# tataganesh/Query-Efficient-Approx-to-improve-OCR

Hardware: AMD Instinct MI355X
Metric: patch-images/sec UNet->CRNN->CTC fwd+bwd, 32x128 grey (higher is better)
Workload: dtype f32 (GEMMs as scaled 2 x fp16 split products — three fp16 MFMAs per fp32 multiply-add — fp32 accumulate); 1 GPU; BASELINE configs[2]: full minibatch step of train_nn_area.py:212-287 — Phase A (UNet eval fwd, TopKCER k = 5 % of the minibatch, inner_limit = 4 jitter replicas fused in the batch dim, CRNN train-BN fwd+bwd, Adam(CRNN)) + Phase B (UNet train-BN -> CRNN BN-eval -> CTC mean + MSE -> backward -> Adam(UNet)) + greedy decode -> CER -> update_cer (:290-304) on synthetic POS-style 32x128 patches; batch_per_gpu=2048, global_batch=2048, full_step=True, crnn_wgrad=True, parallelism=dp1, hipgraph=False

## Files before the change

query-efficient-approx-to-improve-ocr_amd/csrc/conv_igemm.hip:

```cpp
#include "conv_args.h"
#include <string>
#include <type_traits>
#include <stdlib.h>
#include <string.h>

using qea_conv::ConvArgs;
using qea_conv::conv_epilogue;

namespace {

template <int A_LD, int B_LD, int BK, int RPP>
struct IgemmGather {
  int lrow, kc, ntaps;
  int a_pix[A_LD];
  int a_ih0[A_LD], a_iw0[A_LD];
  const float* b_ptr[B_LD > 0 ? B_LD : 1];
  f32x4 a_reg[A_LD], b_reg[B_LD > 0 ? B_LD : 1];

  __device__ __forceinline__ void init(const ConvArgs& p, int tid, int m0, int n0) {
    constexpr int KCH = BK / 4;
    lrow = tid / KCH;
    kc = tid % KCH;
    ntaps = p.KH * p.KW;
    const int ohw = p.OH * p.OW;
#pragma unroll
    for (int i = 0; i < A_LD; ++i) {
      const int m = m0 + lrow + RPP * i;
      if (m < p.M) {
        const int b = m / ohw;
        const int rem = m - b * ohw;
        const int oh = rem / p.OW;
        const int ow = rem - oh * p.OW;
        a_pix[i] = b * p.H * p.W;
        a_ih0[i] = oh * p.stride_h - p.pad_h;
        a_iw0[i] = ow * p.stride_w - p.pad_w;
      } else {
        a_pix[i] = -1;
        a_ih0[i] = 0;
        a_iw0[i] = 0;
      }
    }
#pragma unroll
    for (int j = 0; j < B_LD; ++j) {
      const int n = n0 + lrow + RPP * j;
      b_ptr[j] = (n < p.N) ? (p.w + (size_t)n * p.K + kc * 4) : nullptr;
    }
  }

  __device__ __forceinline__ void fetch(const ConvArgs& p, int kt) {
    const int cs = kt / ntaps;
    const int tap = kt - cs * ntaps;
    const int c0 = cs * BK;
    const int kh = tap / p.KW;
    const int kw = tap - kh * p.KW;
#pragma unroll
    for (int i = 0; i < A_LD; ++i) {
      const int ih = a_ih0[i] + kh, iw = a_iw0[i] + kw;
      const bool ok = (a_pix[i] >= 0) && ((unsigned)ih < (unsigned)p.H) && ((unsigned)iw < (unsigned)p.W);
      f32x4 v = {0.f, 0.f, 0.f, 0.f};
      if (ok) v = *reinterpret_cast<const f32x4*>(p.x + (size_t)(a_pix[i] + ih * p.W + iw) * p.ldx + c0 + kc * 4);
      a_reg[i] = v;
    }
    const int koff = tap * p.Cin + c0;
#pragma unroll
    for (int j = 0; j < B_LD; ++j) {
      f32x4 v = {0.f, 0.f, 0.f, 0.f};
      if (b_ptr[j]) v = *reinterpret_cast<const f32x4*>(b_ptr[j] + koff);
      b_reg[j] = v;
    }
  }
};

template <int MI, int NJ>
__device__ __forceinline__ void zero_acc(f32x16 (&acc)[MI][NJ]) {
#pragma unroll
  for (int i = 0; i < MI; ++i)
#pragma unroll
    for (int j = 0; j < NJ; ++j)
#pragma unroll
      for (int r = 0; r < 16; ++r) acc[i][j][r] = 0.f;
}

constexpr int ROWB = 16;
// ... 646 lines not shown
#pragma unroll
        for (int i = 0; i < MI; ++i)
#pragma unroll
          for (int j = 0; j < NJ; ++j)
            acc[i][j] = __builtin_amdgcn_mfma_f32_32x32x2f32(af[i][s], bq[cur][kb][j][s], acc[i][j], 0, 0, 0);
    }
  }

  float esc[NJ], ebi[NJ];
#pragma unroll
  for (int j = 0; j < NJ; ++j) {
    esc[j] = scale ? scale[j * 32 + fr] : 1.f;
    ebi[j] = bias ? bias[j * 32 + fr] : 0.f;
  }
  double st0[NJ], st1[NJ];
  if (STATS) {
#pragma unroll
    for (int j = 0; j < NJ; ++j) st0[j] = st1[j] = 0.0;
  }
  float am = 0.f;
#pragma unroll
  for (int i = 0; i < MI; ++i) {
    float* yrow = y + ((size_t)(b * H + y0 + wave * MI + i) * W + x0) * ldy;
#pragma unroll
    for (int r = 0; r < 16; ++r) {
      const int px = (r & 3) + 8 * (r >> 2) + 4 * fh;
#pragma unroll
      for (int j = 0; j < NJ; ++j) {
        float v = acc[i][j][r];
        if (scale && bias) v = __fmaf_rn(v, esc[j], ebi[j]);
        else if (scale) v *= esc[j];
        else if (bias) v += ebi[j];
        if (relu) v = fmaxf(v, 0.f);
        yrow[(size_t)px * ldy + j * 32 + fr] = v;
        am = qea_amax_acc(am, v);
        if (STATS) {
          st0[j] += (double)v;
          st1[j] += (double)v * (double)v;
        }
      }
    }
  }
  qea_amax_commit_block(am, yamax);
  if (STATS) {
#pragma unroll
    for (int j = 0; j < NJ; ++j) {
      const double a = st0[j] + __shfl_xor(st0[j], 32, 64);
      const double c = st1[j] + __shfl_xor(st1[j], 32, 64);
      if (fh == 0) {
        double* dst = stats + ((size_t)(blockIdx.x * 4 + wave) * COUT + j * 32 + fr) * 2;
        dst[0] = a;
        dst[1] = c;
      }
    }
  }
}

template <int CIN, int COUT, int TH, bool STATS>
int launch_halo_(const ConvArgs& a, hipStream_t s) {
  constexpr size_t lds = (size_t)(TH + 2) * 34 * (CIN + 4) * sizeof(float);
  constexpr auto kern = conv3x3_halo_kernel<CIN, COUT, TH, STATS>;
  const int rc = reserve_lds<kern>("qea_conv_igemm(halo)", lds);
  if (rc != QEA_OK) return rc;
  const long long grid = (long long)a.B * (a.H / TH) * (a.W / 32);
  if (grid <= 0 || grid > 0x7fffffffLL) {
    qea_set_error("qea_conv_igemm(halo): grid %lld out of range", grid);
    return QEA_ERR_INVALID;
  }
  hipLaunchKernelGGL(kern, dim3((unsigned)grid), dim3(256), lds, s, a.x, a.w, a.y, a.B, a.H, a.W, a.ldx, a.ldy, a.scale, a.bias, a.relu, a.stats, a.yamax);
  return QEA_OK;
}

template <int CIN, int COUT, int TH>
int launch_halo(const ConvArgs& a, hipStream_t s) {
  return a.stats ? launch_halo_<CIN, COUT, TH, true>(a, s) : launch_halo_<CIN, COUT, TH, false>(a, s);
}

#ifndef QEA_HALO_NARROW_WGS
#define QEA_HALO_NARROW_WGS 3
#endif
constexpr int halo_bf3_wgs(int cin, int cout, int npl, bool bst = false) {
  return (npl == 2 && cout <= 64 && (cin == 32 || cout == 32) && !(bst && cout == 64) && QEA_HALO_NARROW_WGS == 3) ? 3 : 2;
}

template <int CIN, int COUT, int TH, bool STATS, int IMW = 0, int NPL = 3, int PKW = 0, bool BST = false>
__global__ __launch_bounds__(256) __attribute__((amdgpu_waves_per_eu(halo_bf3_wgs(CIN, COUT, NPL, BST), halo_bf3_wgs(CIN, COUT, NPL, BST)))) void conv3x3_halo_bf3_kernel(const float* __restrict__ x, const __bf16* __restrict__ wf, float* __restrict__ y,
                                                               int B, int H, int W, int ldx, int ldy, const float* __restrict__ scale,
                                                               const float* __restrict__ bias, int relu, double* __restrict__ stats, int chunks,
                                                               int Ntot, const float* __restrict__ mask, int ldmask, int total,
                                                               const float* __restrict__ xmax, float* __restrict__ yamax,
                                                               float* __restrict__ pooled, int ldp, float* __restrict__ pamax,
                                                               const float* __restrict__ yref, int ldyref, const double* __restrict__ bst64,
                                                               const float* __restrict__ bsc, const float* __restrict__ bsh) {
  constexpr bool F16 = NPL == 2;
  typedef typename std::conditional<F16, f16x8, bf16x8>::type frag_t;
  constexpr bool SMALL = IMW != 0;
  constexpr int IMH = SMALL ? IMW / 4 : 1;
  constexpr int IPX = SMALL ? 32 / IMW : 1, IPY = SMALL ? TH / IMH : 1;
  constexpr int TW = 32, HW_ = SMALL ? IPX * (IMW + 2) : TW + 2, HH = SMALL ? TH + 1 : TH + 2, HP = HH * HW_;
  static_assert(!SMALL || (TH % IMH == 0 && COUT == 128), "small-image tiles: whole images per tile, one wave row");
  constexpr int WN = COUT / 32, WM = 4 / WN;
  constexpr int MI = TH / WM;
  constexpr int KS = CIN / 16;
  constexpr int SLOTS = CIN / 8;
  constexpr int PLANE = HP * CIN;
  static_assert(MI >= 1 && TH % WM == 0, "tile rows must split over the waves");
  static_assert(PKW == 0 || (MI % 2 == 0 && !STATS && (PKW == 1 || PKW == 2)), "fused pooling: row pairs inside one wave, no statistics");
  static_assert(!BST || (!STATS && PKW == 0), "BatchNorm-backward sums: their own instances");
  extern __shared__ __attribute__((aligned(16))) float smem[];
  __bf16* As = reinterpret_cast<__bf16*>(smem);
  float sx = 1.f, inv_x = 1.f, inv_w = 1.f;
  if constexpr (F16) {
    qea_f16_scale(xmax[0], sx, inv_x);
    inv_w = reinterpret_cast<const float*>(wf + (size_t)Ntot * 9 * chunks * CIN * NPL)[0];
  }

  const int tiles_x = W / TW, tiles_y = H / TH;
  const int nblk = Ntot / COUT;
  struct Item { int nb, tile_id, b, x0, y0; };
  auto decode = [&](int vb) {
    const int lid = qea_xcd_swizzle(vb, total);
    Item it;
    it.nb = lid % nblk;
    it.tile_id = lid / nblk;
    if (SMALL) {
      it.b = it.tile_id * (IPX * IPY);
      it.x0 = it.y0 = 0;
      return it;
    }
    int bid = it.tile_id;
    const int tx = bid % tiles_x;
    bid /= tiles_x;
    const int ty = bid % tiles_y;
    it.b = bid / tiles_y;
    it.x0 = tx * TW;
    it.y0 = ty * TH;
    return it;
  };

  auto swz = [](int p, int slot) { return SLOTS == 4 ? (slot ^ ((p >> 2) & 3)) : (slot ^ ((p >> 1) & 7)); };

  constexpr int C4 = CIN / 4;
  constexpr int NLD = (HP * C4 + 255) / 256;
  f32x4 hv[NLD];
  constexpr int QS = 256 / C4;
  auto gather = [&](const Item& it, int chunk, int tid) {
    const float* xb = x + (size_t)it.b * H * W * ldx + chunk * CIN + (tid % C4) * 4;
    int q = tid / C4;
    int hy = q / HW_, hx = q - hy * HW_;
#pragma unroll
    for (int i = 0; i < NLD; ++i) {
      int iy, ix;
      bool ok;
      if (SMALL) {
        const int gx = hx / (IMW + 2);
        const int img = (hy / IMH) * IPX + gx;
        ix = hx - gx * (IMW + 2) - 1;
        iy = (img * IMH + hy % IMH);
        ok = q < HP && hy < TH && (unsigned)ix < (unsigned)IMW && it.b + img < B;
      } else {
        iy = it.y0 + hy - 1;
        ix = it.x0 + hx - 1;
        ok = q < HP && (unsigned)iy < (unsigned)H && (unsigned)ix < (unsigned)W;
      }
      const f32x4 v = *reinterpret_cast<const f32x4*>(ok ? xb + ((size_t)iy * W + ix) * ldx : x);
      const f32x4 zero = {0.f, 0.f, 0.f, 0.f};
      hv[i] = ok ? v : zero;
      q += QS;
      hx += QS;
      if (hx >= HW_) {
        hx -= HW_;
        ++hy;
      }
    }
  };
  auto stage = [&](int tid) {
    const int c4 = tid % C4;
    int q = tid / C4;
#pragma unroll
    for (int i = 0; i < NLD; ++i) {
      if (q < HP) {
        const int o = q * CIN + swz(q, c4 >> 1) * 8 + (c4 & 1) * 4;
        if constexpr (F16) {
          f16x4 h, l;
          qea_split2_f16(hv[i], sx, h, l);
          *reinterpret_cast<f16x4*>(As + o) = h;
          *reinterpret_cast<f16x4*>(As + PLANE + o) = l;
        } else {
          bf16x4 h, m, l;
          qea_split3(hv[i], h, m, l);
          *reinterpret_cast<bf16x4*>(As + o) = h;
          *reinterpret_cast<bf16x4*>(As + PLANE + o) = m;
          *reinterpret_cast<bf16x4*>(As + 2 * PLANE + o) = l;
        }
      }
      q += QS;
    }
  };

  constexpr int STEPS = 9 * KS;
  frag_t bq[2][NPL];
  auto load_b = [&](int nb, int gst, int buf, int tid) {
    const frag_t* wl = reinterpret_cast<const frag_t*>(wf) + ((tid >> 6) % WN) * 64 + (tid & 63) + (size_t)nb * chunks * STEPS * NPL * WN * 64;
#pragma unroll
    for (int pl = 0; pl < NPL; ++pl) bq[buf][pl] = wl[(size_t)(gst * NPL + pl) * WN * 64];
  };

  int vb = blockIdx.x;
  Item cur = decode(vb);
  gather(cur, 0, threadIdx.x);
  load_b(cur.nb, 0, 0, threadIdx.x);
  bool first = true;
  float am = 0.f, pm = 0.f;
  while (true) {
    const int nvb = vb + gridDim.x;
    const bool has_next = nvb < total;
    const Item nxt = decode(has_next ? nvb : vb);
    f32x16 acc[MI];
#pragma unroll
    for (int i = 0; i < MI; ++i)
#pragma unroll
      for (int r = 0; r < 16; ++r) acc[i][r] = 0.f;

    for (int chunk = 0; chunk < chunks; ++chunk) {
      int tid = threadIdx.x;
      asm volatile("" : "+v"(tid));
      const int lane = tid & 63, wave = tid >> 6;
      const int wm = wave / WN;
      const int fr = lane & 31, fh = lane >> 5;
      if (!first) __syncthreads();
      first = false;
      stage(tid);
      __syncthreads();
      if (chunk + 1 < chunks) gather(cur, chunk + 1, tid);
      else if (has_next) gather(nxt, 0, tid);
      auto read_a = [&](int st, int i, frag_t* a) {
        const int tap = st / KS, cs = st % KS;
        const int kh = tap / 3, kw = tap % 3;
        int hp;
        if (SMALL) {
          const int rr = i % IMH + kh - 1;
          const int srow = (rr >= 0 && rr < IMH) ? (i / IMH) * IMH + rr : TH;
          hp = srow * HW_ + fr + 2 * (fr / IMW) + kw;
        } else {
          hp = (wm * MI + i + kh) * HW_ + fr + kw;
        }
        const __bf16* src = As + hp * CIN + swz(hp, cs * 2 + fh) * 8;
#pragma unroll
        for (int pl = 0; pl < NPL; ++pl) a[pl] = *reinterpret_cast<const frag_t*>(src + pl * PLANE);
      };
      frag_t ar[2][NPL];
      read_a(0, 0, ar[0]);
#pragma unroll
      for (int st = 0; st < STEPS; ++st) {
        const int cb = st & 1;
        if (st + 1 < STEPS || chunk + 1 < chunks) load_b(cur.nb, chunk * STEPS + st + 1, cb ^ 1, tid);
        else if (has_next) load_b(nxt.nb, 0, cb ^ 1, tid);
        __builtin_amdgcn_sched_barrier(0);
#pragma unroll
        for (int i = 0; i < MI; ++i) {
          const int f = st * MI + i;
          const bool more = f + 1 < STEPS * MI;
          if (more) read_a((f + 1) / MI, (f + 1) % MI, ar[(f + 1) & 1]);
          acc[i] = mfma_split<NPL>(acc[i], ar[f & 1], bq[cb]);
          if (more) {
            __builtin_amdgcn_sched_group_barrier(0x100, NPL, 0);
            __builtin_amdgcn_sched_group_barrier(0x008, NPL == 2 ? 3 : 6, 0);
          }
        }
      }
    }

    int tid = threadIdx.x;
    asm volatile("" : "+v"(tid));
    const int lane = tid & 63, wave = tid >> 6;
    const int wm = wave / WN, wn = wave % WN;
    const int fr = lane & 31, fh = lane >> 5;
    const int n = cur.nb * COUT + wn * 32 + fr;
    const float esc = scale ? scale[n] : 1.f, ebi = bias ? bias[n] : 0.f;
    float msc = 0.f, msh = 0.f;
    double bmu = 0.0, bis = 0.0;
    if constexpr (BST) {
      msc = bsc[n];
      msh = bsh[n];
      bmu = bst64[n];
      bis = bst64[Ntot + n];
    }
    double st0 = 0.0, st1 = 0.0;
    if constexpr (PKW != 0) {
#pragma unroll
      for (int i = 0; i < MI; i += 2) {
        float vv[2][16];
#pragma unroll
        for (int ii = 0; ii < 2; ++ii)
#pragma unroll
          for (int r = 0; r < 16; ++r) {
            const int px = (r & 3) + 8 * (r >> 2) + 4 * fh;
            size_t prow;
            bool live = true;
            if (SMALL) {
              const int img = ((i + ii) / IMH) * IPX + px / IMW;
              prow = ((size_t)(cur.b + img) * IMH + (i + ii) % IMH) * IMW + px % IMW;
              live = cur.b + img < B;
            } else {
              prow = (size_t)(cur.b * H + cur.y0 + wm * MI + i + ii) * W + cur.x0 + px;
            }
            float v = acc[i + ii][r];
            if constexpr (F16) v = (v * inv_x) * inv_w;
            if (scale && bias) v = __fmaf_rn(v, esc, ebi);
            else if (scale) v *= esc;
            else if (bias) v += ebi;
            if (relu) v = fmaxf(v, 0.f);
            vv[ii][r] = v;
            if (!live) continue;
            y[prow * ldy + n] = v;
            am = qea_amax_acc(am, v);
          }
#pragma unroll
        for (int r = 0; r < 16; r += PKW) {
          const int px = (r & 3) + 8 * (r >> 2) + 4 * fh;
          float m = -INFINITY;
#pragma unroll
          for (int ii = 0; ii < 2; ++ii)
#pragma unroll
            for (int jj = 0; jj < PKW; ++jj) {
              const float v = vv[ii][r + jj];
              m = (v > m || v != v) ? v : m;
            }
          size_t prow;
          bool live = true;
          if (SMALL) {
            const int img = (i / IMH) * IPX + px / IMW;
            prow = ((size_t)(cur.b + img) * (IMH / 2) + (i % IMH) / 2) * (IMW / PKW) + (px % IMW) / PKW;
            live = cur.b + img < B;
          } else {
            prow = ((size_t)cur.b * (H / 2) + (cur.y0 + wm * MI + i) / 2) * (W / PKW) + (cur.x0 + px) / PKW;
          }
          if (!live) continue;
          pooled[prow * ldp + n] = m;
          pm = qea_amax_acc(pm, m);
        }
      }
    } else if constexpr (BST) {
#pragma unroll
      for (int i = 0; i < MI; ++i) {
#pragma unroll
        for (int r = 0; r < 16; ++r) {
          const int px = (r & 3) + 8 * (r >> 2) + 4 * fh;
          size_t prow;
          bool live = true;
          if (SMALL) {
            const int img = (i / IMH) * IPX + px / IMW;
            prow = ((size_t)(cur.b + img) * IMH + i % IMH) * IMW + px % IMW;
            live = cur.b + img < B;
          } else {
            prow = (size_t)(cur.b * H + cur.y0 + wm * MI + i) * W + cur.x0 + px;
          }
          float v = acc[i][r];
          if constexpr (F16) v = (v * inv_x) * inv_w;
          if (scale && bias) v = __fmaf_rn(v, esc, ebi);
          else if (scale) v *= esc;
          else if (bias) v += ebi;
          if (relu) v = fmaxf(v, 0.f);
          if (!live) continue;
          if (mask) v = (mask[prow * ldmask + n] > 0.f) ? v : 0.f;
          y[prow * ldy + n] = v;
          am = qea_amax_acc(am, v);
          const float yv = yref[prow * ldyref + n];
          const float dz = __fmaf_rn(yv, msc, msh) > 0.f ? v : 0.f;
          st0 += (double)dz;
          st1 += (double)dz * (((double)yv - bmu) * bis);
        }
      }
    } else {
      if constexpr (F16) {
#pragma unroll
        for (int i = 0; i < MI; ++i)
#pragma unroll
          for (int r = 0; r < 16; ++r) acc[i][r] = (acc[i][r] * inv_x) * inv_w;
      }
      if (scale && bias) {
#pragma unroll
        for (int i = 0; i < MI; ++i)
#pragma unroll
          for (int r = 0; r < 16; ++r) acc[i][r] = __fmaf_rn(acc[i][r], esc, ebi);
      } else if (scale) {
#pragma unroll
        for (int i = 0; i < MI; ++i)
#pragma unroll
          for (int r = 0; r < 16; ++r) acc[i][r] *= esc;
      } else if (bias) {
#pragma unroll
        for (int i = 0; i < MI; ++i)
#pragma unroll
          for (int r = 0; r < 16; ++r) acc[i][r] += ebi;
      }
      if (relu) {
#pragma unroll
        for (int i = 0; i < MI; ++i)
#pragma unroll
          for (int r = 0; r < 16; ++r) acc[i][r] = fmaxf(acc[i][r], 0.f);
      }
      auto store_rows = [&](auto has_mask) {
        constexpr bool HAS_MASK = decltype(has_mask)::value;
#pragma unroll
        for (int i = 0; i < MI; ++i) {
          const int rowpix = (cur.b * H + cur.y0 + wm * MI + i) * W + cur.x0;
          float* yb = y + (size_t)rowpix * ldy;
          const float* mb = HAS_MASK ? mask + (size_t)rowpix * ldmask : nullptr;
          const int lo = 4 * fh * ldy + n, lom = 4 * fh * ldmask + n;
#pragma unroll
          for (int r = 0; r < 16; ++r) {
            const int c = (r & 3) + 8 * (r >> 2);
            float v = acc[i][r];
            size_t prow = 0;
            if (SMALL) {
              const int px = c + 4 * fh;
              const int img = (i / IMH) * IPX + px / IMW;
              prow = ((size_t)(cur.b + img) * IMH + i % IMH) * IMW + px % IMW;
              if (cur.b + img >= B) continue;
              if (HAS_MASK) v = (mask[prow * ldmask + n] > 0.f) ? v : 0.f;
              y[prow * ldy + n] = v;
            } else {
              if (HAS_MASK) v = (mb[lom + c * ldmask] > 0.f) ? v : 0.f;
              yb[lo + c * ldy] = v;
            }
            am = qea_amax_acc(am, v);
            if (STATS) {
              st0 += (double)v;
              st1 += (double)v * (double)v;
            }
          }
        }
      };
      if (mask) store_rows(std::true_type{});
      else store_rows(std::false_type{});
    }
    if (STATS || BST) {
      const double sa = st0 + __shfl_xor(st0, 32, 64);
      const double sc = st1 + __shfl_xor(st1, 32, 64);
      if (fh == 0) {
        double* dst = stats + ((size_t)(cur.tile_id * WM + wm) * Ntot + n) * 2;
        dst[0] = sa;
        dst[1] = sc;
      }
    }
    if (!has_next) break;
    cur = nxt;
    vb = nvb;
  }
  qea_amax_commit_block(am, yamax);
  if constexpr (PKW != 0) qea_amax_commit_block(pm, pamax);
}

template <int CIN, int COUT, int TH, bool STATS, int IMW = 0, int NPL = 3, int PKW = 0, bool BST = false>
int launch_halo_bf3_(const ConvArgs& a, hipStream_t s) {
  constexpr size_t lds = IMW ? (size_t)NPL * (TH + 1) * (32 / IMW) * (IMW + 2) * CIN * 2 : (size_t)NPL * (TH + 2) * 34 * CIN * 2;
  constexpr auto kern = conv3x3_halo_bf3_kernel<CIN, COUT, TH, STATS, IMW, NPL, PKW, BST>;
  const int rc = reserve_lds<kern>("qea_conv_igemm(halo bf3)", lds);
  if (rc != QEA_OK) return rc;
  const long long total = IMW ? (long long)qea_cdiv(a.B, (32 / IMW) * (TH / (IMW / 4))) * (a.N / COUT)
                              : (long long)a.B * (a.H / TH) * (a.W / 32) * (a.N / COUT);
  if (total <= 0 || total > 0x7fffffffLL) {
    qea_set_error("qea_conv_igemm(halo bf3): grid %lld out of range", total);
    return QEA_ERR_INVALID;
  }
  const int resident = qea_persistent_grid(halo_bf3_wgs(CIN, COUT, NPL, BST));
  const unsigned grid = (total > resident && COUT > 32) ? (unsigned)resident : (unsigned)total;
  hipLaunchKernelGGL(kern, dim3(grid), dim3(256), lds, s, a.x, (const __bf16*)a.wp, a.y, a.B, a.H, a.W, a.ldx, a.ldy,
                     a.scale, a.bias, a.relu, a.stats, a.Cin / CIN, a.N, a.mask, a.ldmask, (int)total, a.xmax, a.yamax, a.pool_y, a.ldpool, a.pool_amax,
                     a.bst_y, a.ldbst, a.bst64, a.bst_scale, a.bst_shift);
  return QEA_OK;
}

template <int CIN, int COUT, int TH, int IMW = 0>
int launch_halo_bf3(const ConvArgs& a, hipStream_t s) {
  if constexpr (CIN == 32) {
    if (a.xmax && a.bst_y)
      return launch_halo_bf3_<CIN, COUT, TH, false, IMW, 2, 0, true>(a, s);
    if (a.xmax)
      return a.stats ? launch_halo_bf3_<CIN, COUT, TH, true, IMW, 2>(a, s) : launch_halo_bf3_<CIN, COUT, TH, false, IMW, 2>(a, s);
  }
  return a.stats ? launch_halo_bf3_<CIN, COUT, TH, true, IMW>(a, s) : launch_halo_bf3_<CIN, COUT, TH, false, IMW>(a, s);
}

bool halo_eligible(const qea_conv_desc* d) {
  const bool ch = (d->Cin == 32 || d->Cin == 64) && (d->N == 32 || d->N == 64);
  const int th = d->Cin == 32 ? 8 : 4;
  return ch && d->KH == 3 && d->KW == 3 && d->pad_h == 1 && d->pad_w == 1 && d->stride_h == 1 && d->stride_w == 1 && d->OH == d->H &&
         d->OW == d->W && d->W % 32 == 0 && d->H % th == 0 && d->out_mode == QEA_OUT_NHWC && !d->mask && !d->accumulate;
}

int halo_bf3_small(const qea_conv_desc* d) {
  if (d->Cin % 64 || d->Cin > 512 || d->N % 128) return 0;
  if (d->W == 16 && d->H == 4) return 16;
  if (d->W == 8 && d->H == 2) return 8;
  return 0;
}

bool halo_bf3_eligible(const qea_conv_desc* d) {
  const bool cin = d->Cin == 32 || (d->Cin % 64 == 0 && d->Cin <= 512);
  const bool cout = d->N == 32 || d->N == 64 || d->N % 128 == 0;
  const int th = d->Cin == 32 ? 8 : 4;
  const bool shape = (d->W % 32 == 0 && d->H % th == 0) || halo_bf3_small(d) != 0;
  return cin && cout && d->KH == 3 && d->KW == 3 && d->pad_h == 1 && d->pad_w == 1 && d->stride_h == 1 && d->stride_w == 1 && d->OH == d->H &&
         d->OW == d->W && shape && d->out_mode == QEA_OUT_NHWC && !d->accumulate;
}

long long halo_bf3_tiles(const qea_conv_desc* d) {
  const int sm = halo_bf3_small(d);
  if (sm) return qea_cdiv(d->B, (32 / sm) * (4 / (sm / 4)));
  return (long long)d->B * (d->H / (d->Cin == 32 ? 8 : 4)) * (d->W / 32);
}

bool halo_bf3_pool_shape(const qea_conv_desc* d, int kw) {
  if (!halo_bf3_eligible(d) || d->mask || d->stats || d->H % 2 || (kw != 1 && kw != 2) || (kw == 2 && d->W % 2)) return false;
  const int sm = halo_bf3_small(d);
  if (sm == 16) return kw == 2;
  if (sm) return false;
  if (d->Cin == 32) return d->N == 32 && kw == 2;
  if (d->N == 64) return kw == 2;
  return d->N % 128 == 0;
}

int launch_halo_bf3_any(const qea_conv_desc* d, const ConvArgs& a, hipStream_t s) {
  const int sm = halo_bf3_small(d);
  if (a.pool_y) return launch_halo_bf3_<32, 32, 8, false, 0, 2, 2>(a, s);
  if (sm == 16) return launch_halo_bf3<64, 128, 4, 16>(a, s);
  if (sm == 8) return launch_halo_bf3<64, 128, 4, 8>(a, s);
  if (d->Cin == 32) {
    if (d->N == 32) return launch_halo_bf3<32, 32, 8>(a, s);
    if (d->N == 64) return launch_halo_bf3<32, 64, 8>(a, s);
    return launch_halo_bf3<32, 128, 8>(a, s);
  }
  if (d->N == 32) return launch_halo_bf3<64, 32, 4>(a, s);
  if (d->N == 64) return launch_halo_bf3<64, 64, 4>(a, s);
  return launch_halo_bf3<64, 128, 4>(a, s);
}

int halo_bf3_wm(const qea_conv_desc* d) { return 4 / ((d->N > 128 ? 128 : d->N) / 32); }

int launch_halo_any(const qea_conv_desc* d, const ConvArgs& a, hipStream_t s) {
  if (d->Cin == 32 && d->N == 32) return launch_halo<32, 32, 8>(a, s);
  if (d->Cin == 32 && d->N == 64) return launch_halo<32, 64, 8>(a, s);
  if (d->Cin == 64 && d->N == 32) return launch_halo<64, 32, 4>(a, s);
  return launch_halo<64, 64, 4>(a, s);
}

// ... 283 lines not shown
```

Measured before the change: 22250 patch-images/s.

## Add producer-consumer warp-specialized halo conv kernel with LDS-resident filters

Adds a new 512-thread persistent kernel for 3x3 convolutions with 32 input channels, 32 or 64 output channels and 8-row tiles. Half the threads gather and stage input halos into a two-slot LDS ring with a three-deep register prefetch, while the other half run the MFMA loop and epilogue. Filter fragments are preloaded once into LDS instead of being streamed from global memory. The epilogue is factored into a shared helper. The path is taken automatically when the work exceeds one persistent wave of blocks and no pooling or BN-backward fusion is requested. It trades occupancy (one 512-thread block per CU) and extra LDS for overlap of global loads with MFMA compute.

```diff
diff --git a/query-efficient-approx-to-improve-ocr_amd/csrc/conv_igemm.hip b/query-efficient-approx-to-improve-ocr_amd/csrc/conv_igemm.hip
--- a/query-efficient-approx-to-improve-ocr_amd/csrc/conv_igemm.hip
+++ b/query-efficient-approx-to-improve-ocr_amd/csrc/conv_igemm.hip
@@ -1,4 +1,5 @@
 #include "conv_args.h"
+#include "item_walk.h"
 #include <string>
 #include <type_traits>
 #include <stdlib.h>
@@ -811,6 +812,45 @@
 constexpr int halo_bf3_wgs(int cin, int cout, int npl, bool bst = false) {
   return (npl == 2 && cout <= 64 && (cin == 32 || cout == 32) && !(bst && cout == 64) && QEA_HALO_NARROW_WGS == 3) ? 3 : 2;
 }
+
+struct HaloItem { int nb, tile_id, b, x0, y0; };
+template <int TH>
+__device__ __forceinline__ HaloItem halo_decode(int vb, int total, int nblk, int tiles_x, int tiles_y) {
+  const int lid = qea_xcd_swizzle(vb, total);
+  HaloItem it;
+  it.nb = lid % nblk;
+  it.tile_id = lid / nblk;
+  int bid = it.tile_id;
+  const int tx = bid % tiles_x;
+  bid /= tiles_x;
+  const int ty = bid % tiles_y;
+  it.b = bid / tiles_y;
+  it.x0 = tx * 32;
+  it.y0 = ty * TH;
+  return it;
+}
+template <int SLOTS>
+__device__ __forceinline__ int halo_swz(int p, int slot) { return SLOTS == 4 ? (slot ^ ((p >> 2) & 3)) : (slot ^ ((p >> 1) & 7)); }
+
+struct HaloEpilogue {
+  float* y;
+  int B, H, W, ldy;
+  const float *scale, *bias;
+  int relu;
+  double* stats;
+  int Ntot;
+  const float* mask;
+  int ldmask;
+  float inv_x, inv_w;
+  float* pooled;
+  int ldp;
+  const float* yref;
+  int ldyref;
+  const double* bst64;
+  const float *bsc, *bsh;
+};
+template <int COUT, int TH, bool STATS, int IMW, int NPL, int PKW, bool BST, int MI>
+__device__ __forceinline__ void halo_bf3_epilogue(f32x16 (&acc)[MI], const HaloItem& cur, const HaloEpilogue& e, float& am, float& pm);
 
 template <int CIN, int COUT, int TH, bool STATS, int IMW = 0, int NPL = 3, int PKW = 0, bool BST = false>
 __global__ __launch_bounds__(256) __attribute__((amdgpu_waves_per_eu(halo_bf3_wgs(CIN, COUT, NPL, BST), halo_bf3_wgs(CIN, COUT, NPL, BST)))) void conv3x3_halo_bf3_kernel(const float* __restrict__ x, const __bf16* __restrict__ wf, float* __restrict__ y,
@@ -846,28 +886,21 @@
 
   const int tiles_x = W / TW, tiles_y = H / TH;
   const int nblk = Ntot / COUT;
-  struct Item { int nb, tile_id, b, x0, y0; };
+  typedef HaloItem Item;
   auto decode = [&](int vb) {
-    const int lid = qea_xcd_swizzle(vb, total);
-    Item it;
-    it.nb = lid % nblk;
-    it.tile_id = lid / nblk;
     if (SMALL) {
+      const int lid = qea_xcd_swizzle(vb, total);
+      Item it;
+      it.nb = lid % nblk;
+      it.tile_id = lid / nblk;
       it.b = it.tile_id * (IPX * IPY);
       it.x0 = it.y0 = 0;
       return it;
     }
-    int bid = it.tile_id;
-    const int tx = bid % tiles_x;
-    bid /= tiles_x;
-    const int ty = bid % tiles_y;
-    it.b = bid / tiles_y;
-    it.x0 = tx * TW;
-    it.y0 = ty * TH;
-    return it;
+    return halo_decode<TH>(vb, total, nblk, tiles_x, tiles_y);
   };
 
-  auto swz = [](int p, int slot) { return SLOTS == 4 ? (slot ^ ((p >> 2) & 3)) : (slot ^ ((p >> 1) & 7)); };
+  auto swz = [](int p, int slot) { return halo_swz<SLOTS>(p, slot); };
 
   constexpr int C4 = CIN / 4;
   constexpr int NLD = (HP * C4 + 255) / 256;
@@ -941,6 +974,7 @@
   load_b(cur.nb, 0, 0, threadIdx.x);
   bool first = true;
   float am = 0.f, pm = 0.f;
+  const HaloEpilogue epi = {y, B, H, W, ldy, scale, bias, relu, stats, Ntot, mask, ldmask, inv_x, inv_w, pooled, ldp, yref, ldyref, bst64, bsc, bsh};
   while (true) {
     const int nvb = vb + gridDim.x;
     const bool has_next = nvb < total;
@@ -1000,186 +1034,398 @@
       }
     }
 
-    int tid = threadIdx.x;
-    asm volatile("" : "+v"(tid));
-    const int lane = tid & 63, wave = tid >> 6;
-    const int wm = wave / WN, wn = wave % WN;
-    const int fr = lane & 31, fh = lane >> 5;
-    const int n = cur.nb * COUT + wn * 32 + fr;
-    const float esc = scale ? scale[n] : 1.f, ebi = bias ? bias[n] : 0.f;
-    float msc = 0.f, msh = 0.f;
-    double bmu = 0.0, bis = 0.0;
-    if constexpr (BST) {
-      msc = bsc[n];
-      msh = bsh[n];
-      bmu = bst64[n];
-      bis = bst64[Ntot + n];
-    }
-    double st0 = 0.0, st1 = 0.0;
-    if constexpr (PKW != 0) {
-#pragma unroll
-      for (int i = 0; i < MI; i += 2) {
-        float vv[2][16];
-#pragma unroll
-        for (int ii = 0; ii < 2; ++ii)
-#pragma unroll
-          for (int r = 0; r < 16; ++r) {
-            const int px = (r & 3) + 8 * (r >> 2) + 4 * fh;
-            size_t prow;
-            bool live = true;
-            if (SMALL) {
-              const int img = ((i + ii) / IMH) * IPX + px / IMW;
-              prow = ((size_t)(cur.b + img) * IMH + (i + ii) % IMH) * IMW + px % IMW;
-              live = cur.b + img < B;
-            } else {
-              prow = (size_t)(cur.b * H + cur.y0 + wm * MI + i + ii) * W + cur.x0 + px;
-            }
-            float v = acc[i + ii][r];
-            if constexpr (F16) v = (v * inv_x) * inv_w;
-            if (scale && bias) v = __fmaf_rn(v, esc, ebi);
-            else if (scale) v *= esc;
-            else if (bias) v += ebi;
-            if (relu) v = fmaxf(v, 0.f);
-            vv[ii][r] = v;
-            if (!live) continue;
-            y[prow * ldy + n] = v;
-            am = qea_amax_acc(am, v);
-          }
-#pragma unroll
-        for (int r = 0; r < 16; r += PKW) {
-          const int px = (r & 3) + 8 * (r >> 2) + 4 * fh;
-          float m = -INFINITY;
-#pragma unroll
-          for (int ii = 0; ii < 2; ++ii)
-#pragma unroll
-            for (int jj = 0; jj < PKW; ++jj) {
-              const float v = vv[ii][r + jj];
-              m = (v > m || v != v) ? v : m;
-            }
-          size_t prow;
-          bool live = true;
-          if (SMALL) {
-            const int img = (i / IMH) * IPX + px / IMW;
-            prow = ((size_t)(cur.b + img) * (IMH / 2) + (i % IMH) / 2) * (IMW / PKW) + (px % IMW) / PKW;
-            live = cur.b + img < B;
-          } else {
-            prow = ((size_t)cur.b * (H / 2) + (cur.y0 + wm * MI + i) / 2) * (W / PKW) + (cur.x0 + px) / PKW;
-          }
-          if (!live) continue;
-          pooled[prow * ldp + n] = m;
-          pm = qea_amax_acc(pm, m);
-        }
-      }
-    } else if constexpr (BST) {
-#pragma unroll
-      for (int i = 0; i < MI; ++i) {
+    halo_bf3_epilogue<COUT, TH, STATS, IMW, NPL, PKW, BST>(acc, cur, epi, am, pm);
+    if (!has_next) break;
+    cur = nxt;
+    vb = nvb;
+  }
+  qea_amax_commit_block(am, yamax);
+  if constexpr (PKW != 0) qea_amax_commit_block(pm, pamax);
+}
+
+template <int COUT, int TH, bool STATS, int IMW, int NPL, int PKW, bool BST, int MI>
+__device__ __forceinline__ void halo_bf3_epilogue(f32x16 (&acc)[MI], const HaloItem& cur, const HaloEpilogue& e, float& am, float& pm) {
+  constexpr bool F16 = NPL == 2, SMALL = IMW != 0;
+  constexpr int IMH = SMALL ? IMW / 4 : 1, IPX = SMALL ? 32 / IMW : 1;
+  constexpr int WN = COUT / 32, WM = 4 / WN;
+  static_assert(MI == TH / WM, "one accumulator tile per 32-pixel row of the wave");
+  float* const y = e.y;
+  const int B = e.B, H = e.H, W = e.W, ldy = e.ldy, relu = e.relu, Ntot = e.Ntot, ldmask = e.ldmask, ldp = e.ldp, ldyref = e.ldyref;
+  const float *const scale = e.scale, *const bias = e.bias, *const mask = e.mask, *const yref = e.yref, *const bsc = e.bsc, *const bsh = e.bsh;
+  double* const stats = e.stats;
+  const double* const bst64 = e.bst64;
+  float* const pooled = e.pooled;
+  const float inv_x = e.inv_x, inv_w = e.inv_w;
+  int tid = threadIdx.x;
+  asm volatile("" : "+v"(tid));
+  const int lane = tid & 63, wave = tid >> 6;
+  const int wm = wave / WN, wn = wave % WN;
+  const int fr = lane & 31, fh = lane >> 5;
+  const int n = cur.nb * COUT + wn * 32 + fr;
+  const float esc = scale ? scale[n] : 1.f, ebi = bias ? bias[n] : 0.f;
+  float msc = 0.f, msh = 0.f;
+  double bmu = 0.0, bis = 0.0;
+  if constexpr (BST) {
+    msc = bsc[n];
+    msh = bsh[n];
+    bmu = bst64[n];
+    bis = bst64[Ntot + n];
+  }
+  double st0 = 0.0, st1 = 0.0;
+  if constexpr (PKW != 0) {
+#pragma unroll
+    for (int i = 0; i < MI; i += 2) {
+      float vv[2][16];
+#pragma unroll
+      for (int ii = 0; ii < 2; ++ii)
 #pragma unroll
         for (int r = 0; r < 16; ++r) {
           const int px = (r & 3) + 8 * (r >> 2) + 4 * fh;
           size_t prow;
           bool live = true;
           if (SMALL) {
-            const int img = (i / IMH) * IPX + px / IMW;
-            prow = ((size_t)(cur.b + img) * IMH + i % IMH) * IMW + px % IMW;
+            const int img = ((i + ii) / IMH) * IPX + px / IMW;
+            prow = ((size_t)(cur.b + img) * IMH + (i + ii) % IMH) * IMW + px % IMW;
             live = cur.b + img < B;
           } else {
-            prow = (size_t)(cur.b * H + cur.y0 + wm * MI + i) * W + cur.x0 + px;
+            prow = (size_t)(cur.b * H + cur.y0 + wm * MI + i + ii) * W + cur.x0 + px;
           }
-          float v = acc[i][r];
+          float v = acc[i + ii][r];
           if constexpr (F16) v = (v * inv_x) * inv_w;
           if (scale && bias) v = __fmaf_rn(v, esc, ebi);
           else if (scale) v *= esc;
           else if (bias) v += ebi;
           if (relu) v = fmaxf(v, 0.f);
+          vv[ii][r] = v;
           if (!live) continue;
-          if (mask) v = (mask[prow * ldmask + n] > 0.f) ? v : 0.f;
           y[prow * ldy + n] = v;
           am = qea_amax_acc(am, v);
-          const float yv = yref[prow * ldyref + n];
-          const float dz = __fmaf_rn(yv, msc, msh) > 0.f ? v : 0.f;
-          st0 += (double)dz;
-          st1 += (double)dz * (((double)yv - bmu) * bis);
         }
+#pragma unroll
+      for (int r = 0; r < 16; r += PKW) {
+        const int px = (r & 3) + 8 * (r >> 2) + 4 * fh;
+        float m = -INFINITY;
+#pragma unroll
+        for (int ii = 0; ii < 2; ++ii)
+#pragma unroll
+          for (int jj = 0; jj < PKW; ++jj) {
+            const float v = vv[ii][r + jj];
+            m = (v > m || v != v) ? v : m;
+          }
+        size_t prow;
+        bool live = true;
+        if (SMALL) {
+          const int img = (i / IMH) * IPX + px / IMW;
+          prow = ((size_t)(cur.b + img) * (IMH / 2) + (i % IMH) / 2) * (IMW / PKW) + (px % IMW) / PKW;
+          live = cur.b + img < B;
+        } else {
+          prow = ((size_t)cur.b * (H / 2) + (cur.y0 + wm * MI + i) / 2) * (W / PKW) + (cur.x0 + px) / PKW;
+        }
+        if (!live) continue;
+        pooled[prow * ldp + n] = m;
+        pm = qea_amax_acc(pm, m);
+      }
+    }
+  } else if constexpr (BST) {
+#pragma unroll
+    for (int i = 0; i < MI; ++i) {
+#pragma unroll
+      for (int r = 0; r < 16; ++r) {
+        const int px = (r & 3) + 8 * (r >> 2) + 4 * fh;
+        size_t prow;
+        bool live = true;
+        if (SMALL) {
+          const int img = (i / IMH) * IPX + px / IMW;
+          prow = ((size_t)(cur.b + img) * IMH + i % IMH) * IMW + px % IMW;
+          live = cur.b + img < B;
+        } else {
+          prow = (size_t)(cur.b * H + cur.y0 + wm * MI + i) * W + cur.x0 + px;
+        }
+        float v = acc[i][r];
+        if constexpr (F16) v = (v * inv_x) * inv_w;
+        if (scale && bias) v = __fmaf_rn(v, esc, ebi);
+        else if (scale) v *= esc;
+        else if (bias) v += ebi;
+        if (relu) v = fmaxf(v, 0.f);
+        if (!live) continue;
+        if (mask) v = (mask[prow * ldmask + n] > 0.f) ? v : 0.f;
+        y[prow * ldy + n] = v;
+        am = qea_amax_acc(am, v);
+        const float yv = yref[prow * ldyref + n];
+        const float dz = __fmaf_rn(yv, msc, msh) > 0.f ? v : 0.f;
+        st0 += (double)dz;
+        st1 += (double)dz * (((double)yv - bmu) * bis);
+      }
+    }
+  } else {
+    if constexpr (F16) {
+#pragma unroll
+      for (int i = 0; i < MI; ++i)
+#pragma unroll
+        for (int r = 0; r < 16; ++r) acc[i][r] = (acc[i][r] * inv_x) * inv_w;
+    }
+    if (scale && bias) {
+#pragma unroll
+      for (int i = 0; i < MI; ++i)
+#pragma unroll
+        for (int r = 0; r < 16; ++r) acc[i][r] = __fmaf_rn(acc[i][r], esc, ebi);
+    } else if (scale) {
+#pragma unroll
+      for (int i = 0; i < MI; ++i)
+#pragma unroll
+        for (int r = 0; r < 16; ++r) acc[i][r] *= esc;
+    } else if (bias) {
+#pragma unroll
+      for (int i = 0; i < MI; ++i)
+#pragma unroll
+        for (int r = 0; r < 16; ++r) acc[i][r] += ebi;
+    }
+    if (relu) {
+#pragma unroll
+      for (int i = 0; i < MI; ++i)
+#pragma unroll
+        for (int r = 0; r < 16; ++r) acc[i][r] = fmaxf(acc[i][r], 0.f);
+    }
+    auto store_rows = [&](auto has_mask) {
+      constexpr bool HAS_MASK = decltype(has_mask)::value;
+#pragma unroll
+      for (int i = 0; i < MI; ++i) {
+        const int rowpix = (cur.b * H + cur.y0 + wm * MI + i) * W + cur.x0;
+        float* yb = y + (size_t)rowpix * ldy;
+        const float* mb = HAS_MASK ? mask + (size_t)rowpix * ldmask : nullptr;
+        const int lo = 4 * fh * ldy + n, lom = 4 * fh * ldmask + n;
+#pragma unroll
+        for (int r = 0; r < 16; ++r) {
+          const int c = (r & 3) + 8 * (r >> 2);
+          float v = acc[i][r];
+          size_t prow = 0;
+          if (SMALL) {
+            const int px = c + 4 * fh;
+            const int img = (i / IMH) * IPX + px / IMW;
+            prow = ((size_t)(cur.b + img) * IMH + i % IMH) * IMW + px % IMW;
+            if (cur.b + img >= B) continue;
+            if (HAS_MASK) v = (mask[prow * ldmask + n] > 0.f) ? v : 0.f;
+            y[prow * ldy + n] = v;
+          } else {
+            if (HAS_MASK) v = (mb[lom + c * ldmask] > 0.f) ? v : 0.f;
+            yb[lo + c * ldy] = v;
+          }
+          am = qea_amax_acc(am, v);
+          if (STATS) {
+            st0 += (double)v;
+            st1 += (double)v * (double)v;
+          }
+        }
+      }
+    };
+    if (mask) store_rows(std::true_type{});
+    else store_rows(std::false_type{});
+  }
+  if (STATS || BST) {
+    const double sa = st0 + __shfl_xor(st0, 32, 64);
+    const double sc = st1 + __shfl_xor(st1, 32, 64);
+    if (fh == 0) {
+      double* dst = stats + ((size_t)(cur.tile_id * WM + wm) * Ntot + n) * 2;
+      dst[0] = sa;
+      dst[1] = sc;
+    }
+  }
+}
+
+constexpr int HALO_PC_RING = 2;
+constexpr int HALO_PC_DEPTH = 3;
+constexpr size_t HALO_PC_BUF_BYTES = (size_t)2 * 10 * 34 * 32 * 2;
+constexpr size_t halo_pc_filter_bytes(int cout) { return (size_t)18 * 2 * (cout / 32) * 64 * 16; }
+
+template <int COUT, bool STATS, int PKW, bool BST>
+__global__ __launch_bounds__(512) __attribute__((amdgpu_waves_per_eu(2, 2))) void conv3x3_halo_pc_kernel(
+    const float* __restrict__ x, const __bf16* __restrict__ wf, float* __restrict__ y, int B, int H, int W, int ldx, int ldy,
+    const float* __restrict__ scale, const float* __restrict__ bias, int relu, double* __restrict__ stats, int Ntot,
+    const float* __restrict__ mask, int ldmask, int total, const float* __restrict__ xmax, float* __restrict__ yamax,
+    float* __restrict__ pooled, int ldp, float* __restrict__ pamax, const float* __restrict__ yref, int ldyref,
+    const double* __restrict__ bst64, const float* __restrict__ bsc, const float* __restrict__ bsh) {
+  constexpr int CIN = 32, TH = 8, NPL = 2, TW = 32, HW_ = TW + 2, HP = (TH + 2) * HW_;
+  constexpr int WN = COUT / 32, WM = 4 / WN, MI = TH / WM, KS = CIN / 16, SLOTS = CIN / 8, STEPS = 9 * KS;
+  constexpr int PLANE = HP * CIN, BUF = NPL * PLANE;
+  static_assert(BUF * 2 == HALO_PC_BUF_BYTES, "ring buffer size");
+  static_assert(STEPS % 2 == 0, "the filter fragments' buffer parity carries over items");
+  typedef f16x8 frag_t;
+  extern __shared__ __attribute__((aligned(16))) float smem[];
+  _Float16* ring = reinterpret_cast<_Float16*>(smem);
+  constexpr int WFRAGS = STEPS * NPL * WN * 64;
+  static_assert((size_t)WFRAGS * 16 == halo_pc_filter_bytes(COUT), "filter size in LDS");
+  frag_t* wlds = reinterpret_cast<frag_t*>(ring + HALO_PC_RING * BUF);
+  float sx, inv_x;
+  qea_f16_scale(xmax[0], sx, inv_x);
+  const float inv_w = reinterpret_cast<const float*>(wf + (size_t)Ntot * 9 * CIN * NPL)[0];
+
+  const int tiles_x = W / TW, tiles_y = H / TH, nblk = Ntot / COUT;
+  const qea_item_walk walk = qea_walk(blockIdx.x, gridDim.x, total);
+  const int rounds = qea_walk_rounds(walk);
+  auto item = [&](int k) { return halo_decode<TH>(qea_walk_item(walk, k), total, nblk, tiles_x, tiles_y); };
+  float am = 0.f, pm = 0.f;
+
+  if (walk.count > 0) {
+    const frag_t* src = reinterpret_cast<const frag_t*>(wf);
+    for (int e = threadIdx.x; e < WFRAGS; e += 512) wlds[e] = src[e];
+    __syncthreads();
+  }
+
+  if (threadIdx.x >= 256) {
+    constexpr int C4 = CIN / 4, NLD = (HP * C4 + 255) / 256, QS = 256 / C4;
+    f32x4 hv[HALO_PC_DEPTH][NLD];
+    auto gather = [&](int k, f32x4* h) {
+      const HaloItem it = item(k);
+      int t = threadIdx.x - 256;
+      asm volatile("" : "+v"(t));
+      const float* xb = x + (size_t)it.b * H * W * ldx + (t % C4) * 4;
+      int q = t / C4;
+      int hy = q / HW_, hx = q - hy * HW_;
+      unsigned inside = 0;
+#pragma unroll
+      for (int i = 0; i < NLD; ++i) {
+        const int iy = it.y0 + hy - 1, ix = it.x0 + hx - 1;
+        const bool ok = q < HP && (unsigned)iy < (unsigned)H && (unsigned)ix < (unsigned)W;
+        h[i] = *reinterpret_cast<const f32x4*>(ok ? xb + ((size_t)iy * W + ix) * ldx : x);
+        inside |= ok ? 1u << i : 0u;
+        q += QS;
+        hx += QS;
+        if (hx >= HW_) {
+          hx -= HW_;
+          ++hy;
+        }
+      }
+      return inside;
+    };
+    auto stage = [&](const f32x4* h, unsigned inside, _Float16* As) {
+      int t = threadIdx.x - 256;
+      asm volatile("" : "+v"(t));
+      const int c4 = t % C4;
+      int q = t / C4;
+#pragma unroll
+      for (int i = 0; i < NLD; ++i) {
+        if (q < HP) {
+          const int o = q * CIN + halo_swz<SLOTS>(q, c4 >> 1) * 8 + (c4 & 1) * 4;
+          const f32x4 zero = {0.f, 0.f, 0.f, 0.f};
+          f16x4 hi, lo;
+          qea_split2_f16((inside >> i) & 1u ? h[i] : zero, sx, hi, lo);
+          *reinterpret_cast<f16x4*>(As + o) = hi;
+          *reinterpret_cast<f16x4*>(As + PLANE + o) = lo;
+        }
+        q += QS;
+      }
+    };
+    unsigned in_img[HALO_PC_DEPTH] = {};
+    int r0 = 0;
+    if (walk.count >= 2 * HALO_PC_DEPTH) {
+#pragma unroll
+      for (int d = 0; d < HALO_PC_DEPTH; ++d) in_img[d] = gather(d, hv[d]);
+      for (; r0 + 2 * HALO_PC_DEPTH <= walk.count; r0 += HALO_PC_DEPTH) {
+#pragma unroll
+        for (int d = 0; d < HALO_PC_DEPTH; ++d) {
+          const int r = r0 + d;
+          stage(hv[d], in_img[d], ring + qea_walk_slot(r, HALO_PC_RING) * BUF);
+          in_img[d] = gather(r + HALO_PC_DEPTH, hv[d]);
+          if (qea_walk_barrier_after(walk, r)) __syncthreads();
+        }
       }
     } else {
-      if constexpr (F16) {
+#pragma unroll
+      for (int d = 0; d < HALO_PC_DEPTH; ++d)
+        if (d < walk.count) in_img[d] = gather(d, hv[d]);
+    }
+    for (; r0 < rounds; r0 += HALO_PC_DEPTH) {
+#pragma unroll
+      for (int d = 0; d < HALO_PC_DEPTH; ++d) {
+        const int r = r0 + d;
+        if (r < rounds) {
+          const int k = qea_walk_staged(walk, r);
+          if (k >= 0) {
+            stage(hv[d], in_img[d], ring + qea_walk_slot(k, HALO_PC_RING) * BUF);
+            if (k + HALO_PC_DEPTH < walk.count) in_img[d] = gather(k + HALO_PC_DEPTH, hv[d]);
+          }
+          if (qea_walk_barrier_after(walk, r)) __syncthreads();
+        }
+      }
+    }
+  } else {
+    frag_t bq[2][NPL];
+    auto load_b = [&](int st, int buf, int tid) {
+      const frag_t* wl = wlds + ((tid >> 6) % WN) * 64 + (tid & 63);
+#pragma unroll
+      for (int pl = 0; pl < NPL; ++pl) bq[buf][pl] = wl[(st * NPL + pl) * WN * 64];
+    };
+    const HaloEpilogue epi = {y, B, H, W, ldy, scale, bias, relu, stats, Ntot, mask, ldmask, inv_x, inv_w, pooled, ldp, yref, ldyref, bst64, bsc, bsh};
+    if (walk.count > 0) load_b(0, 0, threadIdx.x);
+    for (int r = 0; r < rounds; ++r) {
+      const int k = qea_walk_computed(walk, r);
+      if (k >= 0) {
+        const HaloItem cur = item(k);
+        const _Float16* As = ring + qea_walk_slot(k, HALO_PC_RING) * BUF;
+        f32x16 acc[MI];
 #pragma unroll
         for (int i = 0; i < MI; ++i)
 #pragma unroll
-          for (int r = 0; r < 16; ++r) acc[i][r] = (acc[i][r] * inv_x) * inv_w;
-      }
-      if (scale && bias) {
-#pragma unroll
-        for (int i = 0; i < MI; ++i)
-#pragma unroll
-          for (int r = 0; r < 16; ++r) acc[i][r] = __fmaf_rn(acc[i][r], esc, ebi);
-      } else if (scale) {
-#pragma unroll
-        for (int i = 0; i < MI; ++i)
-#pragma unroll
-          for (int r = 0; r < 16; ++r) acc[i][r] *= esc;
-      } else if (bias) {
-#pragma unroll
-        for (int i = 0; i < MI; ++i)
-#pragma unroll
-          for (int r = 0; r < 16; ++r) acc[i][r] += ebi;
-      }
-      if (relu) {
-#pragma unroll
-        for (int i = 0; i < MI; ++i)
-#pragma unroll
-          for (int r = 0; r < 16; ++r) acc[i][r] = fmaxf(acc[i][r], 0.f);
-      }
-      auto store_rows = [&](auto has_mask) {
-        constexpr bool HAS_MASK = decltype(has_mask)::value;
-#pragma unroll
-        for (int i = 0; i < MI; ++i) {
-          const int rowpix = (cur.b * H + cur.y0 + wm * MI + i) * W + cur.x0;
-          float* yb = y + (size_t)rowpix * ldy;
-          const float* mb = HAS_MASK ? mask + (size_t)rowpix * ldmask : nullptr;
-          const int lo = 4 * fh * ldy + n, lom = 4 * fh * ldmask + n;
-#pragma unroll
-          for (int r = 0; r < 16; ++r) {
-            const int c = (r & 3) + 8 * (r >> 2);
-            float v = acc[i][r];
-            size_t prow = 0;
-            if (SMALL) {
-              const int px = c + 4 * fh;
-              const int img = (i / IMH) * IPX + px / IMW;
-              prow = ((size_t)(cur.b + img) * IMH + i % IMH) * IMW + px % IMW;
-              if (cur.b + img >= B) continue;
-              if (HAS_MASK) v = (mask[prow * ldmask + n] > 0.f) ? v : 0.f;
-              y[prow * ldy + n] = v;
-            } else {
-              if (HAS_MASK) v = (mb[lom + c * ldmask] > 0.f) ? v : 0.f;
-              yb[lo + c * ldy] = v;
-            }
-            am = qea_amax_acc(am, v);
-            if (STATS) {
-              st0 += (double)v;
-              st1 += (double)v * (double)v;
+          for (int q = 0; q < 16; ++q) acc[i][q] = 0.f;
+        int tid = threadIdx.x;
+        asm volatile("" : "+v"(tid));
+        const int lane = tid & 63, wave = tid >> 6;
+        const int wm = wave / WN;
+        const int fr = lane & 31, fh = lane >> 5;
+        auto read_a = [&](int st, int i, frag_t* a) {
+          const int tap = st / KS, cs = st % KS;
+          const int kh = tap / 3, kw = tap % 3;
+          const int hp = (wm * MI + i + kh) * HW_ + fr + kw;
+          const _Float16* src = As + hp * CIN + halo_swz<SLOTS>(hp, cs * 2 + fh) * 8;
+#pragma unroll
+          for (int pl = 0; pl < NPL; ++pl) a[pl] = *reinterpret_cast<const frag_t*>(src + pl * PLANE);
+        };
+        frag_t ar[2][NPL];
+        read_a(0, 0, ar[0]);
+#pragma unroll
+        for (int st = 0; st < STEPS; ++st) {
+          const int cb = st & 1;
+          load_b((st + 1) % STEPS, cb ^ 1, tid);
+          __builtin_amdgcn_sched_barrier(0);
+#pragma unroll
+          for (int i = 0; i < MI; ++i) {
+            const int f = st * MI + i;
+            const bool more = f + 1 < STEPS * MI;
+            if (more) read_a((f + 1) / MI, (f + 1) % MI, ar[(f + 1) & 1]);
+            acc[i] = mfma_split<NPL>(acc[i], ar[f & 1], bq[cb]);
+            if (more) {
+              __builtin_amdgcn_sched_group_barrier(0x100, NPL, 0);
+              __builtin_amdgcn_sched_group_barrier(0x008, 3, 0);
             }
           }
         }
-      };
-      if (mask) store_rows(std::true_type{});
-      else store_rows(std::false_type{});
-    }
-    if (STATS || BST) {
-      const double sa = st0 + __shfl_xor(st0, 32, 64);
-      const double sc = st1 + __shfl_xor(st1, 32, 64);
-      if (fh == 0) {
-        double* dst = stats + ((size_t)(cur.tile_id * WM + wm) * Ntot + n) * 2;
-        dst[0] = sa;
-        dst[1] = sc;
-      }
-    }
-    if (!has_next) break;
-    cur = nxt;
-    vb = nvb;
+        halo_bf3_epilogue<COUT, TH, STATS, 0, NPL, PKW, BST>(acc, cur, epi, am, pm);
+      }
+      if (qea_walk_barrier_after(walk, r)) __syncthreads();
+    }
   }
   qea_amax_commit_block(am, yamax);
   if constexpr (PKW != 0) qea_amax_commit_block(pm, pamax);
+}
+
+int halo_pc_mode() {
+  const char* e = getenv("QEA_HALO_PC");
+  return (!e || !*e) ? -1 : (e[0] == '0' && !e[1] ? 0 : 1);
+}
+
+constexpr bool halo_pc_auto(int cout, bool stats, int pkw, bool bst) { return !bst && pkw == 0; }
+
+template <int COUT, bool STATS, int PKW, bool BST>
+int launch_halo_pc_(const ConvArgs& a, hipStream_t s, long long total) {
+  constexpr size_t lds = HALO_PC_RING * HALO_PC_BUF_BYTES + halo_pc_filter_bytes(COUT);
+  constexpr auto kern = conv3x3_halo_pc_kernel<COUT, STATS, PKW, BST>;
+  const int rc = reserve_lds<kern>("qea_conv_igemm(halo pc)", lds);
+  if (rc != QEA_OK) return rc;
+  const int grid = qea_persistent_grid(1);
+  hipLaunchKernelGGL(kern, dim3((unsigned)grid), dim3(512), lds, s, a.x, (const __bf16*)a.wp, a.y, a.B, a.H, a.W, a.ldx, a.ldy, a.scale,
+                     a.bias, a.relu, a.stats, a.N, a.mask, a.ldmask, (int)total, a.xmax, a.yamax, a.pool_y, a.ldpool, a.pool_amax, a.bst_y,
+                     a.ldbst, a.bst64, a.bst_scale, a.bst_shift);
+  return QEA_OK;
 }
 
 template <int CIN, int COUT, int TH, bool STATS, int IMW = 0, int NPL = 3, int PKW = 0, bool BST = false>
@@ -1193,6 +1439,11 @@
   if (total <= 0 || total > 0x7fffffffLL) {
     qea_set_error("qea_conv_igemm(halo bf3): grid %lld out of range", total);
     return QEA_ERR_INVALID;
+  }
+  if constexpr (CIN == 32 && TH == 8 && IMW == 0 && NPL == 2 && (COUT == 32 || COUT == 64)) {
+    const int pc = halo_pc_mode();
+    if (a.Cin == CIN && a.N == COUT && (pc == 1 || (pc < 0 && halo_pc_auto(COUT, STATS, PKW, BST) && total > qea_persistent_grid(1))))
+      return launch_halo_pc_<COUT, STATS, PKW, BST>(a, s, total);
   }
   const int resident = qea_persistent_grid(halo_bf3_wgs(CIN, COUT, NPL, BST));
   const unsigned grid = (total > resident && COUT > 32) ? (unsigned)resident : (unsigned)total;
diff --git a/query-efficient-approx-to-improve-ocr_amd/csrc/item_walk.h b/query-efficient-approx-to-improve-ocr_amd/csrc/item_walk.h
--- /dev/null
+++ b/query-efficient-approx-to-improve-ocr_amd/csrc/item_walk.h
@@ -0,0 +1,25 @@
+#pragma once
+
+#if defined(__HIPCC__)
+#define QEA_WALK_FN __host__ __device__ inline
+#else
+#define QEA_WALK_FN inline
+#endif
+
+struct qea_item_walk {
+  int first, stride, count;
+};
+
+QEA_WALK_FN qea_item_walk qea_walk(int wg, int grid, int total) {
+  qea_item_walk w;
+  w.first = wg;
+  w.stride = grid;
+  w.count = total > wg ? (int)(((long long)total - wg + grid - 1) / grid) : 0;
+  return w;
+}
+QEA_WALK_FN int qea_walk_item(const qea_item_walk& w, int k) { return w.first + k * w.stride; }
+QEA_WALK_FN int qea_walk_rounds(const qea_item_walk& w) { return w.count + 1; }
+QEA_WALK_FN int qea_walk_staged(const qea_item_walk& w, int r) { return r < w.count ? r : -1; }
+QEA_WALK_FN int qea_walk_computed(const qea_item_walk& w, int r) { return (r >= 1 && r <= w.count) ? r - 1 : -1; }
+QEA_WALK_FN int qea_walk_slot(int k, int ring) { return k % ring; }
+QEA_WALK_FN bool qea_walk_barrier_after(const qea_item_walk& w, int r) { return r < w.count; }
```

Result: slower. 21810 patch-images/s (-2.0%).
